# data61/gossamer

Measured on AMD Instinct MI355X. Metric: M k-mers/s (canonical, counted) at k=25, 150 bp reads, higher is better.
Workload: dtype u64

## Files before the change

### gossamer_amd/csrc/fused_path.hpp

```cpp
#pragma once

enum { kFusedDeclined = 0, kFusedDone = 1, kFusedNeedFull = 2, kFusedGoOn = -1, kFusedAgain = -2 };
constexpr uint32_t kFusedGrid = 256 * GOSS_E1_OCC;
#ifndef GOSS_FUSED_NKEYS2
#define GOSS_FUSED_NKEYS2 14
#endif
#ifndef GOSS_FUSED_GRID2
#define GOSS_FUSED_GRID2 512
#endif
constexpr uint32_t kFusedGrid2 = GOSS_FUSED_GRID2;
constexpr double kValidSlackA = 1.06, kValidSlackB = 1.17;
constexpr uint64_t kValidSizingMin = 640u << 20;

struct FusedForm {
    enum Table {
        kSmall,
        kBig,
        kWide,
        k96,
        kRem32
    };
    Table table = kSmall;
    uint32_t segbits = kSegBits;
    bool msd = false;
// ... 367 lines not shown
template <class F> void with_digit_hists(int nh, F&& f)
{
    if (nh == 0) f(std::integral_constant<int, 0>{});
    else if (nh == 1) f(std::integral_constant<int, 1>{});
    else f(std::integral_constant<int, 2>{});
}

struct FirstLevelLaunch {
    const uint8_t* d_bases; const uint8_t* aligned; const uint8_t* pk_src; const uint16_t* pk_bad;
    uint32_t mis; uint64_t nstarts, navail;
    void* ka; PartCounters* pc; const GapTable* dgt;
    uint32_t part_shift; uint64_t nsuper; uint32_t blk_log2, grid;
    int nh;
};

template <int MODE, int REPK>
void launch_extract1_part(goss_gpu_ctx* c, const FirstLevelLaunch& a, bool fastk, bool narrow, uint32_t nr_rbits, uint32_t nr_sqbit, uint32_t nr_dmask,
                          uint32_t nr_capg)
{
    with_digit_hists(a.nh, [&](auto nh_c) { with_bool(fastk, [&](auto fast_c) { with_bool(narrow, [&](auto narrow_c) {
        constexpr int NH = decltype(nh_c)::value;
        constexpr bool FAST = NH == 0 && decltype(fast_c)::value, NRW = NH == 0 && decltype(narrow_c)::value;
        if (c->rec_mode)
            hipLaunchKernelGGL(HIP_KERNEL_NAME(extract1_part_kernel<MODE, NH, REPK, true, FAST, NRW>), dim3(a.grid), dim3(kTB), 0, c->stream,
                               a.d_bases, 0u, a.nstarts, a.nstarts / rec_slots(c), c->len, (Key1*)a.ka, a.pc, a.dgt, a.part_shift, a.nsuper, a.blk_log2,
                               nr_rbits, nr_sqbit, nr_dmask, nr_capg);
        else if (c->pk.on)
            hipLaunchKernelGGL(HIP_KERNEL_NAME(extract1_part_kernel<MODE, NH, REPK, false, FAST, NRW, true>), dim3(a.grid), dim3(kTB), 0, c->stream,
                               a.pk_src, a.mis, a.nstarts, a.navail, c->len, (Key1*)a.ka, a.pc, a.dgt, a.part_shift, a.nsuper, a.blk_log2,
                               nr_rbits, nr_sqbit, nr_dmask, nr_capg, a.pk_bad);
        else
            hipLaunchKernelGGL(HIP_KERNEL_NAME(extract1_part_kernel<MODE, NH, REPK, false, FAST, NRW>), dim3(a.grid), dim3(kTB), 0, c->stream,
                               a.aligned, a.mis, a.nstarts, a.navail, c->len, (Key1*)a.ka, a.pc, a.dgt, a.part_shift, a.nsuper, a.blk_log2,
                               nr_rbits, nr_sqbit, nr_dmask, nr_capg, (const uint16_t*)nullptr);
    }); }); });
}

template <int MODE, int NBH>
void launch_extract2_part(goss_gpu_ctx* c, const FirstLevelLaunch& a)
{
    with_digit_hists(a.nh, [&](auto nh_c) {
        constexpr int NH = decltype(nh_c)::value;
        if constexpr (MODE == 0)
            if (c->rec_mode)
            {
                hipLaunchKernelGGL(HIP_KERNEL_NAME(extract2_part_kernel<0, NH, GOSS_FUSED_NKEYS2, NBH, true>), dim3(a.grid), dim3(kTB), 0, c->stream,
                                   a.d_bases, 0u, a.nstarts, a.nstarts / rec_slots(c), c->len, (Key2*)a.ka, a.pc, a.dgt, a.part_shift, a.nsuper, a.blk_log2);
                return;
            }
        if (c->pk.on)
            hipLaunchKernelGGL(HIP_KERNEL_NAME(extract2_part_kernel<MODE, NH, GOSS_FUSED_NKEYS2, NBH, false, true>), dim3(a.grid), dim3(kTB), 0, c->stream,
                               a.pk_src, a.mis, a.nstarts, a.navail, c->len, (Key2*)a.ka, a.pc, a.dgt, a.part_shift, a.nsuper, a.blk_log2, a.pk_bad);
        else
            hipLaunchKernelGGL(HIP_KERNEL_NAME(extract2_part_kernel<MODE, NH, GOSS_FUSED_NKEYS2, NBH>), dim3(a.grid), dim3(kTB), 0, c->stream,
                               a.aligned, a.mis, a.nstarts, a.navail, c->len, (Key2*)a.ka, a.pc, a.dgt, a.part_shift, a.nsuper, a.blk_log2,
                               (const uint16_t*)nullptr);
    });
}

template <class K>
void launch_first_level(const FusedChunk<K>& ch, const FusedForm& form, bool canon_l1, const BucketRegions& br, const GapTable* dgt, PartCounters* pc)
{
    goss_gpu_ctx* c = ch.c;
    const uint32_t shift = ch.keybits - form.segbits, npass = (form.segbits + 7) / 8;
    FirstLevelLaunch a{};
    const uintptr_t addr = (uintptr_t)ch.d_bases;
    a.d_bases = ch.d_bases;
    a.mis = (uint32_t)(addr & 15u);
    a.aligned = (const uint8_t*)(addr - a.mis);
    if (c->pk.on && !c->rec_mode) { pk_ptrs(c, a.aligned, &a.pk_src, &a.pk_bad); c->pk_fused_chunks++; }
    a.nstarts = ch.nstarts; a.navail = ch.navail;
    a.ka = ch.ka; a.pc = pc; a.dgt = dgt;
    a.part_shift = form.msd ? ch.keybits - 8 : shift;
    a.nsuper = (ch.nstarts + br.super - 1) / br.super;
    a.blk_log2 = br.blk_log2;
    a.grid = br.grid;
    a.nh = form.msd ? 0 : (npass > 2 ? 2 : 1);
    PhaseTimer t(c, GOSS_T_EXTRACT, ch.nstarts);
    if constexpr (FusedChunk<K>::kOne)
    {
        const bool fastk = a.nh == 0 && 2 * c->len >= 32 && a.part_shift >= 34 && !c->no_fast32;
        const bool narrow = form.msd && form.rem32() && form.narrow;
        const uint32_t nr_rbits = form.rbits32, nr_sqbit = form.squeeze ? c->len - 1 : 0u, nr_dmask = (1u << form.r32_bits) - 1u;
        const uint32_t nr_capg = std::min(656u, std::max(576u, c->narrow_capg));
        if (ch.graph_mode) launch_extract1_part<1, 0>(c, a, fastk, narrow, nr_rbits, nr_sqbit, nr_dmask, nr_capg);
        else if (canon_l1) launch_extract1_part<0, 2>(c, a, fastk, narrow, nr_rbits, nr_sqbit, nr_dmask, nr_capg);
        else if (c->len & 1u) launch_extract1_part<0, 1>(c, a, fastk, narrow, nr_rbits, nr_sqbit, nr_dmask, nr_capg);
        else launch_extract1_part<0, 0>(c, a, fastk, narrow, nr_rbits, nr_sqbit, nr_dmask, nr_capg);
    }
    else
    {
        if (ch.graph_mode) launch_extract2_part<1, 8>(c, a);
        else if (ch.rep_graph) launch_extract2_part<0, 0>(c, a);
        else
            switch (key2_nbh(c))
            {
                case 2: launch_extract2_part<0, 2>(c, a); break;
                case 4: launch_extract2_part<0, 4>(c, a); break;
                case 6: launch_extract2_part<0, 6>(c, a); break;
                default: launch_extract2_part<0, 8>(c, a); break;
            }
    }
    t.stop();
}

struct FirstLevelResult { uint64_t n = 0, tiles = 0, windows = 0; };

template <class K>
int read_first_level(const FusedChunk<K>& ch, const FusedForm& form, const BucketRegions& br, const PartCounters* pc, GapTable* gt, GapTable* dgt,
                     FirstLevelResult* out)
{
    goss_gpu_ctx* c = ch.c;
    std::vector<unsigned long long> hpc(sizeof(PartCounters) / 8);
    HIP_TRY(hipMemcpyAsync(hpc.data(), pc, sizeof(PartCounters), hipMemcpyDeviceToHost, c->stream));
    HIP_TRY(hipStreamSynchronize(c->stream));
    const PartCounters* hp = (const PartCounters*)hpc.data();
    if (hp->overflow) { c->fused_overflows++; return ch.decline("a bucket region overflowed"); }
    ch.lap("extraction + first level");
#if defined(GOSS_STAMPS)
    if (hp->hist[505])
        std::fprintf(stderr, "libgossgpu: stamps per tile (cycles): A %.0f  B %.0f  C %.0f  scatter %.0f  D %.0f   (%llu tiles)\n",
                     (double)hp->hist[500] / hp->hist[505], (double)hp->hist[501] / hp->hist[505], (double)hp->hist[502] / hp->hist[505],
                     (double)hp->hist[503] / hp->hist[505], (double)hp->hist[504] / hp->hist[505], (unsigned long long)hp->hist[505]);
    if (hp->hist[505] && hp->hist[506])
        std::fprintf(stderr, "libgossgpu: stamps, finer: C = scan %.0f + bookkeeping %.0f + barrier; scatter = LDS %.0f + encoder %.0f + barrier; D = stores %.0f + absorb %.0f + barrier %.0f\n",
                     (double)hp->hist[506] / hp->hist[505], (double)hp->hist[507] / hp->hist[505], (double)hp->hist[510] / hp->hist[505],
                     (double)hp->hist[511] / hp->hist[505], (double)hp->hist[508] / hp->hist[505], (double)hp->hist[509] / hp->hist[505],
                     (double)hp->hist[504] / hp->hist[505]);
#endif
    const uint64_t n = hp->keys_out;
    if (n == 0) return kFusedDeclined;
    if (n > ch.ka_slots || n > ch.kb_slots) return ch.decline("more keys than the buffers hold");
    const bool narrow = form.rem32() && form.narrow;
    uint64_t tiles = 0, sum = 0;
    const uint64_t tile_keys = narrow ? (uint64_t)(form.r32_bits == 9 ? Sub32N<9>::kTileSlots : Sub32N<10>::kTileSlots)
                             : form.rem32() ? (uint64_t)kSub32Tile : form.msd ? (uint64_t)SubCfg<K>::kTile : (uint64_t)SortCfg<K, false>::kTile;
    for (int d = 0; d < 256; ++d)
    {
        gt->cnt[d] = hp->cursors[d * kCursorStride];
        gt->tile_first[d] = tiles;
        tiles += (gt->cnt[d] + tile_keys - 1) / tile_keys;
        sum += gt->cnt[d];
    }
    gt->tile_first[256] = tiles;
    const uint64_t n_slots = narrow ? n / 3 * 2 : n;
    const uint64_t B = 1ULL << br.blk_log2;
    if (sum < n_slots || sum > n_slots + 8 + (uint64_t)br.grid * 256 * (2 * B + 8))
        throw StatusError{GOSS_ERR_HIP, "fused extraction: bucket counts do not add up"};
    HIP_TRY(hipMemcpyAsync(dgt, gt, sizeof(GapTable), hipMemcpyHostToDevice, c->stream));
    out->n = n; out->tiles = tiles; out->windows = hp->windows;
    return kFusedGoOn;
}

struct FusedLookback { LookbackCtl* ctl; LookbackCtl* hctl; };

inline int count_rem32(const FusedChunk<Key1>& ch, FusedForm form, const Sub32Regions& sub, const FirstLevelResult& fl, const GapTable* dgt,
                       FusedLookback lb, Run* r)
{
    goss_gpu_ctx* c = ch.c;
    Key1* ka = ch.ka; Key1* kb = ch.kb;
    const uint64_t n = fl.n, tiles = fl.tiles;
    const uint32_t r32_regions = form.r32_regions(), r32_bits = form.r32_bits, r32_split = form.r32_split, rbits32 = form.rbits32;
    const uint32_t sqbit32 = c->len - 1;
    const bool narrow = form.narrow, squeeze = form.squeeze;
    const bool image = r32_split == 0;
    if (squeeze && (rbits32 != kNarrowSqRbits || r32_bits != kNarrowSqDigitBits))
        throw StatusError{GOSS_ERR_HIP, "fused path: the squeeze form with other than 33-bit remainders under nine second-level bits"};
// ... 316 lines not shown
```

### gossamer_amd/csrc/goss_gpu.hip

```cpp
#include "../../include/goss_gpu.h"

#include <hip/hip_runtime.h>
#include <dlfcn.h>

#include <algorithm>
#include <chrono>
#include <cmath>
#include <cstdio>
#include <cstdlib>
#include <cstring>
#include <functional>
#include <map>
#include <mutex>
#include <string>
#include <system_error>
#include <thread>
#include <vector>

#include "goss_kernels.hpp"
#include "goss_reader.hpp"

using namespace goss;

namespace {
// ... 35 lines not shown
    void release(uint64_t m) { hi = m; }
    uint64_t avail() const { return hi > lo ? hi - lo : 0; }
};

struct OutFile {
    std::string suffix;
    uint64_t size = 0;
    const uint8_t* dev = nullptr;
    std::vector<uint8_t> host;
};

typedef std::map<std::pair<uint64_t, uint64_t>, uint64_t> BigMap;
struct Run { void* keys; uint32_t* counts; uint64_t m; int big = -1; bool rep = false; };

struct PhaseEvents { hipEvent_t a, b; int phase; uint64_t units; };

enum class Held : uint8_t { None, Segments, Entries, Components };
struct HeldResult { Held kind = Held::None; uint64_t lo = 0; };

constexpr double kCanonL1At = 0.05;
constexpr int kBigRoundsMax = 2;

}

struct goss_gpu_ctx {
    int device = 0;
    uint32_t k = 0, len = 0;
    int mode = 0;
    int words = 1;
    int path = 0;
    bool lookback = true;
    double est_scale = 1.0;
    uint32_t order_bits = 0;
    bool ordered_tiles = false;
    uint32_t lookback_failures = 0;
    uint64_t emit_estimate = 0;
    bool has_emit_estimate = false;
    struct Pending { hipEvent_t ev; void (*fn)(void*); void* user; };
    std::vector<Pending> pending;
    uint64_t flush_wait_us = 0, flush_count_us = 0, flushes = 0;
    struct PackedSrc { bool on = false; const uint32_t* codes = nullptr; const uint16_t* bad = nullptr; } pk;
    bool stage_pk[2] = {false, false};
    uint8_t* stage_buf[2] = {nullptr, nullptr};
    int stage_cur = 0;
    hipStream_t copy_stream = nullptr;
    std::thread bg;
    int bg_status = GOSS_OK;
    std::string bg_error;
    std::vector<hipEvent_t> pend_pool;
    uint8_t* stage = nullptr;
    uint64_t stage_cap = 0, stage_fill = 0;
    bool mute_timing = false;
    uint32_t segment_retries = 0;
    uint32_t extract_hist_shift = 0xFFFFFFFFu;
    bool extract_rep = false;
    uint32_t rep_chunks = 0;
    bool graph_rep = true;
    int canon_l1 = 1;
    bool more_follows = false;
    uint64_t more_starts = 0;
    uint64_t expect_bases = 0;
    int space_choice = -1;
    uint32_t canon_chunks = 0;
    bool fused = true;
    uint64_t fused_min = 32u << 20;
    uint32_t fused_overflows = 0;
    uint32_t valid_sized_chunks = 0;
    uint32_t valid_resizes = 0;
    uint64_t dump_lo = 0;
    bool dump_live = false;
    uint64_t budget_limit = 0;
    uint32_t arena_grows = 0;
    uint64_t arena_ms = 0;
    std::thread arena_thread;
    int arena_status = GOSS_OK;
    std::string arena_error;
    uint32_t seg_merges = 0;
    uint32_t hash_merges = 0;
    uint64_t hash_merge_min = 1u << 20;
    bool fused_msd = true;
    uint32_t fused_msd_chunks = 0;
    bool rem32 = true;
    int rem32_slots = 0;
    uint32_t narrow_capg = 656;
    bool narrow = true;
    uint32_t r32_small_max = 0;
    bool overflow_by_sort = true;
    uint64_t overflow_units = 0;
    uint32_t rem32_chunks = 0;
    uint32_t narrow_chunks = 0;
    uint64_t assemble_us = 0;
    uint64_t ds_blocks_ranges = 0, ds_blocks_own = 0;
    uint32_t pk_fused_chunks = 0;
    uint32_t pk_unpacked_chunks = 0;
    uint32_t rem32_bits_min = 0;
    uint32_t rem32_bits_last = 0;
    uint32_t rem32_split_min = 0;
    uint32_t rem32_split_last = 0;
    uint32_t fused_chunks = 0;
    bool debug = false;
    double fused_capscale = 1.0;
    uint32_t blk_log2_max = 0;
    bool no_fast32 = false;
    bool table96 = true;
    uint32_t table96_chunks = 0;
    bool wide_table = true;
    bool big_table = true;
    int big_rounds_min = 0;
    uint32_t big_table_chunks = 0;
    uint32_t wide_table_chunks = 0;
    bool rec_mode = false;
    uint32_t rec_chunks = 0;
    bool deferred = false;
    uint8_t* grp_send = nullptr;
    uint64_t grp_send_cap = 0;
    uint8_t* grp_inbox = nullptr;
    uint64_t grp_inbox_cap = 0;
    hipStream_t xstream = nullptr;
    double valid_frac = 1.0;
    bool size_by_valid = true;
    uint64_t budget = 0;
    hipStream_t stream = nullptr;
    bool own_stream = false;
    std::string last_error;
    Arena arena;
    std::vector<Run> runs;
    std::vector<BigMap> big_maps;
    BigMap res_big;
    bool pushed_counts = false;
    uint64_t windows = 0, keys_total = 0;
    bool finished = false, emitted = false;
    bool broken = false;
    double grp_count_ms = 0;
    void* res_keys = nullptr;
    uint32_t* res_counts = nullptr;
    uint64_t M = 0;
    void* tips_keys = nullptr;
    uint32_t* tips_counts = nullptr;
    HeldResult held;
    bool keep_held = false;
    void* seg_recs = nullptr;
    uint8_t* seg_text = nullptr;
    uint64_t seg_count = 0, seg_text_bytes = 0;
    uint32_t* cmp_marks = nullptr;
    uint64_t cmp_mark_words = 0, cmp_built_lo = 0, cmp_marked = 0;
    uint32_t* cmp_labels = nullptr;
    void* cmp_recs = nullptr;
    uint64_t cmp_count = 0;
    bool cmp_built = false;
    std::vector<OutFile> files;
    ExtractCounters* d_ctr = nullptr;
    uint32_t* d_flags = nullptr;
    void* d_route = nullptr;
    void* h_pinned = nullptr;
    std::vector<PhaseEvents> events;
    std::vector<hipEvent_t> event_pool;
    goss_gpu_timing timing{};
};

namespace {

struct PhaseTimer {
    goss_gpu_ctx* c;
    PhaseEvents pe;
    PhaseTimer(goss_gpu_ctx* ctx, int phase, uint64_t units = 0) : c(ctx)
    {
        muted = c->mute_timing;
// ... 5004 lines not shown
```

### gossamer_amd/csrc/kernels_extract.hpp

```cpp
#pragma once
#include <type_traits>

#include <hip/hip_runtime.h>
#include <stdint.h>

#include "goss_key.hpp"
#include "kernels_common.hpp"
#include "goss_words.hpp"

namespace goss {


struct ExtractCounters {
    unsigned long long keys_out;
    unsigned long long windows;
    unsigned long long hist[512];
};

template <bool PACKED = false>
__global__ __launch_bounds__(kTB) void nonbase_sample_kernel(const uint8_t* __restrict__ aligned, uint64_t nslices,
                                                             uint64_t stride, uint32_t slice,
                                                             unsigned long long* __restrict__ out)
{
    unsigned long long bad = 0, seen = 0;
// ... 343 lines not shown
        for (int g = 0; g < G; ++g)
        {
            const uint32_t vm = vmask[g];
            if (vm)
            {
                const uint32_t q0 = (g * kTB + tid) * P + mis;
                const uint32_t v0 = q0 >> 4, sh = q0 & 15u;
                const uint64_t w0 = (uint64_t)pk[v0] | ((uint64_t)pk[v0 + 1] << 32);
                const uint64_t w1 = (uint64_t)pk[v0 + 2] | ((uint64_t)pk[v0 + 3] << 32);
                const uint64_t w2 = (uint64_t)pk[v0 + 4] | ((uint64_t)pk[v0 + 5] << 32);
                uint32_t s = slot[g] * S;
                Key2 f{0, 0};
#pragma unroll
                for (int i = 0; i < P; ++i)
                {
                    const uint32_t t2 = 2 * (sh + i);
                    Key2 e;
                    e.lo = t2 ? ((w0 >> t2) | (w1 << (64 - t2))) : w0;
                    e.hi = (t2 ? ((w1 >> t2) | (w2 << (64 - t2))) : w1) & mask_hi;
                    if (i == 0)
                    {
                        const uint64_t rlo = rev64(e.hi), rhi = rev64(e.lo);
                        const uint32_t sft = 128 - bits;
                        if (sft == 64) { f.lo = rhi; f.hi = 0; }
                        else { f.lo = (rlo >> sft) | (rhi << (64 - sft)); f.hi = rhi >> sft; }
                    }
                    else
                    {
                        const uint32_t pos = 2 * (sh + i + len - 1);
                        const uint64_t nb = (pos < 64 ? (w0 >> pos) : pos < 128 ? (w1 >> (pos - 64)) : (w2 >> (pos - 128))) & 3u;
                        f.hi = ((f.hi << 2) | (f.lo >> 62)) & mask_hi;
                        f.lo = (f.lo << 2) | nb;
                    }
                    if ((vm >> i) & 1u)
                    {
                        const Key2 rk{~e.lo, (~e.hi) & mask_hi};
                        if (MODE == 0) { if constexpr (NBH == 0) stage[s++] = strand_rep2(f, rk, len, lmask); else stage[s++] = canonical_tail<NBH>(f, rk); }
                        else { stage[s++] = f; stage[s++] = rk; }
                    }
                }
            }
            __syncthreads();
            const uint32_t nk = sub_cnt[g] * S;
            for (uint32_t i = tid; i < nk; i += kTB) out[ob + i] = stage[i];
            ob += nk;
            __syncthreads();
        }
    }
}


constexpr int kCursorStride = 32;

struct GapTable {
    unsigned long long reg_start[256];
    unsigned long long reg_cap[256];
    unsigned long long cnt[256];
    unsigned long long tile_first[257];
};

struct PartCounters {
    unsigned long long keys_out, windows, overflow, pad;
    unsigned long long hist[512];
    unsigned long long cursors[256 * kCursorStride];
};

constexpr int kSubCursorStride = 4;
struct SubTable {
    unsigned long long start[65536];
    unsigned long long cap[65536];
};

constexpr uint64_t kPadKey = ~0ULL;

constexpr uint32_t kSkPadWord2 = 1u << 27;
__host__ __device__ inline uint32_t rec_windows(uint32_t w2) { return (w2 >> 27) == 1u ? 0u : (w2 >> 28) + 1u; }
#ifndef GOSS_E1_NK
#define GOSS_E1_NK 16
#endif
#ifndef GOSS_E1_OCC
#define GOSS_E1_OCC 3
#endif
#ifndef GOSS_E1_NCH
#define GOSS_E1_NCH 4
#endif
#ifndef GOSS_E1_PRIO_C
#define GOSS_E1_PRIO_C 1
#define GOSS_E1_PRIO_S 2
#define GOSS_E1_PRIO_E 1
#define GOSS_E1_PRIO_D 3
#endif
__device__ __forceinline__ uint32_t bit_select(uint32_t mask, uint32_t ones, uint32_t zeros)
{
    uint32_t d;
    asm("v_bfi_b32 %0, %1, %2, %3" : "=v"(d) : "v"(mask), "v"(ones), "v"(zeros));
    return d;
}
template <int MODE, int NH, int REPK, bool REC = false, bool FAST = false, bool NARROW = false, bool PACKED = false>
__global__ __launch_bounds__(kTB, GOSS_E1_OCC) void extract1_part_kernel(const uint8_t* __restrict__ bases_aligned, uint32_t mis,
                                                            uint64_t nstarts, uint64_t navail, uint32_t len,
                                                            Key1* __restrict__ out, PartCounters* __restrict__ pc,
                                                            const GapTable* __restrict__ gt, uint32_t shift, uint64_t nsuper,
                                                            uint32_t blk_log2, uint32_t nr_rbits = 0, uint32_t nr_sqbit = 0, uint32_t nr_dmask = 0, uint32_t nr_capg = 0,
                                                            const uint16_t* __restrict__ pbad = nullptr)
{
    static_assert(!(PACKED && REC), "records are not bases");
    static_assert(!NARROW || NH == 0, "the narrow form is the two-level form's");
    constexpr int S = MODE == 1 ? 2 : 1;
    constexpr int P = GOSS_E1_NK / S;
#if !defined(GOSS_E1_EXPERIMENT)
    static_assert(!REC || GOSS_E1_NK == 16, "a record of 16 windows holds at most one thread's first window");
#endif
    constexpr int T = kTB * P;
    constexpr int NVEC = T / 16 + 4;
    constexpr int NK = P * S;
    constexpr int kCarry = NARROW ? 11 : 7;
    constexpr uint32_t kGran = NARROW ? 12 : 8;
    constexpr uint32_t kSlots = NARROW ? 656 * 12 : T * S + 256 * kCarry;
    static_assert(kSlots % kGran == 0 && kSlots >= T * S + 256 * kCarry, "whole granules, and room for a tile without carried keys");
    constexpr uint32_t kGarb = kSlots;
    constexpr int kPairs = GOSS_E1_NK >= 16 ? 5 : 3;
    constexpr uint32_t kStep = 2 * kPairs * kTB;
    constexpr uint32_t kNG = NARROW ? 772 : kSlots / kGran + 4;
    constexpr uint32_t kSkip = 0xFFFFFFFFu;
    constexpr uint32_t kSortedBytes = NARROW ? (kSlots + 128) * 6 : (kSlots + 128) * 8;
    constexpr uint32_t kDigBase = (kSlots + 128) * 4;
    static_assert(kDigBase % 16 == 0, "the digit array starts on a 16-byte boundary");
    __shared__ __attribute__((aligned(64))) unsigned char lds_all[kSortedBytes + (288 + 288 + kNG + 8 + (NH ? 256 * NH : 0)) * 4];
    Key1* const sorted = reinterpret_cast<Key1*>(lds_all);
    uint32_t* const dh = reinterpret_cast<uint32_t*>(lds_all + kSortedBytes);
    uint32_t* const tab = dh + 288;
    uint32_t* const gaddr = tab + 288;
    uint32_t* const sh_scan = gaddr + kNG;
    uint32_t& sh_ovf = sh_scan[6];
    uint32_t* const lh = sh_scan + 8;
    uint32_t* pk = reinterpret_cast<uint32_t*>(sorted);
    uint32_t* iv = pk + NVEC;

    const uint32_t tid = threadIdx.x;
    if (NH > 0) lh[tid] = 0;
    if (NH > 1) lh[tid + 256] = 0;
    dh[tid] = 0;
    if (tid < 32) { dh[256 + tid] = 0; tab[256 + tid] = kGarb << (NARROW ? 2 : 3); }
    if (tid == 0) { sh_ovf = 0; gaddr[kSlots / kGran] = kSkip; }
    const uint64_t my_start = gt->reg_start[tid], my_cap = gt->reg_cap[tid];
    const uint32_t B = 1u << blk_log2;
    const uint32_t bits = 2 * len;
    const uint64_t kmask = (1ULL << bits) - 1;
    const uint64_t lmask = (1ULL << len) - 1;
    unsigned long long nvalid = 0;
    uint64_t wpos = 0;
    uint32_t ccnt = 0;
    Key1 kc[NARROW ? 1 : kCarry];
#pragma unroll
    for (int j = 0; j < (NARROW ? 1 : kCarry); ++j) kc[j].lo = 0;
    uint4 clo0 = make_uint4(0, 0, 0, 0), clo1 = clo0, clo2 = clo0;
    uint64_t cdig0 = 0, cdig1 = 0, cdig2 = 0;
    [[maybe_unused]] auto store_short_granule = [&](Key1* at) {
        const uint32_t lw[12] = {clo0.x, clo0.y, clo0.z, clo0.w, clo1.x, clo1.y, clo1.z, clo1.w, clo2.x, clo2.y, clo2.z, clo2.w};
        const uint64_t dw[3] = {cdig0, cdig1, cdig2};
        uint4* const g = reinterpret_cast<uint4*>(at);
#pragma unroll
        for (int c = 0; c < 4; ++c)
        {
            const uint32_t nv = ccnt > (uint32_t)c + 8 ? 3u : ccnt > (uint32_t)c + 4 ? 2u : ccnt > (uint32_t)c ? 1u : 0u;
            const uint32_t da = (uint32_t)(dw[c / 4] >> (16 * (c % 4))) & 0x3FFu;
            const uint32_t db = (uint32_t)(dw[(c + 4) / 4] >> (16 * ((c + 4) % 4))) & 0x3FFu;
            const uint32_t dc = (uint32_t)(dw[(c + 8) / 4] >> (16 * ((c + 8) % 4))) & 0x3FFu;
            g[c] = make_uint4(lw[c], lw[c + 4], lw[c + 8], da | (db << 10) | (dc << 20) | (nv << 30));
        }
    };

    auto fetch = [&](uint64_t byte0, uint4& q) -> bool {
        if constexpr (PACKED)
        {
            q = make_uint4(0u, 0xFFFFu, 0u, 0u);
            if (byte0 < navail + mis)
            {
                const uint64_t g = byte0 >> 4;
                q.x = reinterpret_cast<const uint32_t*>(bases_aligned)[g];
                q.y = pbad[g];
                const uint64_t left = navail + mis - byte0;
                q.z = left < 16 ? (0xFFFFu << (uint32_t)left) & 0xFFFFu : 0u;
            }
            return true;
        }
        if (byte0 + 16 <= navail + mis) { q = *reinterpret_cast<const uint4*>(bases_aligned + byte0); return true; }
        q = make_uint4(0x0A0A0A0Au, 0x0A0A0A0Au, 0x0A0A0A0Au, 0x0A0A0A0Au);
        if (byte0 < navail + mis)
        {
            uint32_t w[4] = {q.x, q.y, q.z, q.w};
            for (int j = 0; j < 16; ++j)
            {
                uint64_t b = byte0 + j;
                uint32_t c = b < navail + mis ? bases_aligned[b] : 0x0Au;
                w[j >> 2] = (w[j >> 2] & ~(0xFFu << (8 * (j & 3)))) | (c << (8 * (j & 3)));
            }
            q = make_uint4(w[0], w[1], w[2], w[3]);
        }
        return true;
    };
    auto encode = [](const uint4& q, uint32_t& codes, uint32_t& bads) {
        if constexpr (PACKED) { codes = q.x; bads = q.y | q.z; return; }
        const uint32_t w[4] = {q.x, q.y, q.z, q.w};
        codes = 0; bads = 0;
#pragma unroll
        for (int i = 0; i < 4; ++i)
        {
            uint32_t bad;
            const uint32_t x = base_codes(w[i], bad);
            codes |= pack_codes(x) << (8 * i);
            bads |= pack_flags(bad) << (4 * i);
        }
    };
    constexpr uint32_t NV0 = T / 16;
    static_assert(NVEC == NV0 + 4 && NV0 <= kTB, "one vector per thread and four more");
    uint32_t c0 = 0, b0 = 0, c1 = 0, b1 = 0;
    const uint32_t* recw = reinterpret_cast<const uint32_t*>(bases_aligned);
    const uint64_t nrec = navail;
    uint64_t rc_next = 0, rc_end = 0;
    uint32_t ra0 = 0, ra1 = 0, ra2 = kSkPadWord2, rb0 = 0, rb1 = 0, rb2 = kSkPadWord2;
    uint32_t* rbuf = pk;
    uint32_t* rmark = pk + 512 * 8;
    auto stage_rec = [&](uint32_t at, uint32_t x0, uint32_t x1, uint32_t x2, uint32_t before) {
        const uint32_t x2m = x2 & 0x0FFFFFFFu, nw = (x2 >> 28) + 1u;
        if constexpr (!(MODE == 0 && REPK == 1))
        {
// ... 209 lines not shown
#pragma unroll
                for (int i = 0; i < P; ++i)
                {
                    const uint32_t t2 = 30u - r_s2;
                    const uint32_t rlo = __builtin_amdgcn_alignbit(rc1, rc0, r_s2) & kmlo, rhi = __builtin_amdgcn_alignbit(rc2, rc1, r_s2) & kmhi;
                    const uint32_t flo = __builtin_amdgcn_alignbit(rv1, rv0, t2) & kmlo, fhi = __builtin_amdgcn_alignbit(rv2, rv1, t2) & kmhi;
                    if (MODE == 0 && REPK == 1)
                    {
                        const uint32_t sel = (uint32_t)__builtin_amdgcn_sbfe((int32_t)flo, len - 1u, 1u);
                        kreg[i].lo = ((uint64_t)bit_select(sel, rhi, fhi) << 32) | bit_select(sel, rlo, flo);
                    }
                    else emit(i, ((uint64_t)fhi << 32) | flo, ((uint64_t)rhi << 32) | rlo);
                    if (i + 1 < P)
                    {
                        r_s2 += 2u;
                        if (r_s2 >= r_nw2 && r_at < 511) next_rec();
                    }
                }
            }
            else if constexpr (FAST)
            {
                constexpr bool kLoose = MODE == 0 && REPK == 1 && NARROW && NH == 0;
                [[maybe_unused]] const uint32_t kmhi = (uint32_t)(kmask >> 32);
                const uint32_t cw0 = ~(uint32_t)blo, cw1 = ~(uint32_t)(blo >> 32), cw2 = ~(uint32_t)bhi;
                const uint32_t pn = bits - 2;
                const uint32_t nx = (uint32_t)((blo >> pn) | (bhi << (64 - pn)));
                const uint32_t mid = (uint32_t)(blo >> (len - 1));
                const uint64_t f0 = rev64(blo & kmask) >> (64 - bits);
                uint32_t flo = (uint32_t)f0, fhi = (uint32_t)(f0 >> 32);
#pragma unroll
                for (int i = 0; i < P; ++i)
                {
                    if (i)
                    {
                        const uint32_t nb = (nx >> (2 * i)) & 3u;
                        fhi = __builtin_amdgcn_alignbit(fhi, flo, 30);
                        if constexpr (!kLoose) fhi &= kmhi;
                        flo = (flo << 2) | nb;
                    }
                    const uint32_t rlo = i ? __builtin_amdgcn_alignbit(cw1, cw0, 2 * i) : cw0;
                    uint32_t rhi = i ? __builtin_amdgcn_alignbit(cw2, cw1, 2 * i) : cw1;
                    if constexpr (!kLoose) rhi &= kmhi;
                    if (MODE == 0 && REPK == 1)
                    {
                        const uint32_t sel = (uint32_t)__builtin_amdgcn_sbfe((int32_t)mid, 2 * i, 1);
                        kreg[i].lo = ((uint64_t)bit_select(sel, rhi, fhi) << 32) | bit_select(sel, rlo, flo);
                    }
                    else emit(i, ((uint64_t)fhi << 32) | flo, ((uint64_t)rhi << 32) | rlo);
#pragma unroll
                    for (int u = 0; u < S; ++u) rank_key(i * S + u);
                }
            }
            else
            {
                uint64_t f = rev64(blo & kmask) >> (64 - bits);
                uint64_t r = (~blo) & kmask;
                const uint32_t top = bits - 2;
#pragma unroll
                for (int i = 0; i < P; ++i)
                {
                    if (i)
                    {
                        const uint32_t pos = 2 * (i + len - 1);
                        const uint32_t nb = (uint32_t)(pos < 64 ? (blo >> pos) : (bhi >> (pos - 64))) & 3u;
                        f = ((f << 2) | nb) & kmask;
                        r = (r >> 2) | ((uint64_t)(nb ^ 3u) << top);
                    }
                    emit(i, f, r);
                }
            }
            if constexpr (REC || !FAST)
            {
#pragma unroll
                for (int j = 0; j < NK; ++j) rank_key(j);
            }
        }
        __syncthreads();
        GOSS_STAMP(1);
#if !defined(GOSS_E1_NOPRIO)
        __builtin_amdgcn_s_setprio(GOSS_E1_PRIO_C);
#endif

        uint32_t total_slots = 0, part_at = 0, absorb = 0;
        if constexpr (NARROW)
        {
            const uint32_t cnt = dh[tid];
            uint32_t tot = ccnt + cnt;
            uint32_t fg = (tot * 0xAAABu) >> 19;
            uint32_t rest = tot - 12u * fg;
            uint32_t g_at = block_excl_scan_open_u32(fg + (rest ? 1u : 0u), sh_scan, &total_slots);
            GOSS_STAMP(6);
            dh[tid] = 0;
            if (tid < 32) dh[256 + tid] = 0;
            uint32_t thr, tbx, tby;
            auto take_room = [&](uint32_t fl) {
                const uint32_t room = (B - ((uint32_t)wpos & (B - 1))) & (B - 1);
                thr = fl;
                tbx = (uint32_t)(wpos >> 3);
                tby = 0;
                if (fl > room)
                {
                    thr = room;
                    const uint32_t need = fl - room;
                    unsigned long long at, want;
                    if (has_resv && need <= B) { at = resv; want = B; has_resv = false; }
                    else
                    {
                        want = ((uint64_t)(need + B - 1) >> blk_log2) << blk_log2;
                        at = atomicAdd(&pc->cursors[tid * kCursorStride], want);
                    }
                    if (at + want > my_cap) { atomicOr(&pc->overflow, 1ULL); sh_ovf = 1; }
                    tby = (uint32_t)((my_start + at) >> 3);
                    wpos = my_start + at + need;
                }
                else wpos += fl;
            };
            if (total_slots > nr_capg)
            {
                if (ccnt)
                {
                    take_room(8u);
                    if (sh_ovf == 0) store_short_granule(out + ((uint64_t)(thr ? tbx : tby) << 3));
                    ccnt = 0;
                }
                __syncthreads();
                tot = cnt;
                fg = (tot * 0xAAABu) >> 19;
                rest = tot - 12u * fg;
                g_at = block_excl_scan_open_u32(fg + (rest ? 1u : 0u), sh_scan, &total_slots);
            }
            const uint32_t fl = fg << 3;
            part_at = 12u * (g_at + fg);
            take_room(fl);
            tab[tid] = (12u * g_at + ccnt) << 2;
            {
                const uint32_t t8 = thr >> 3;
                const uint32_t yb = tby - t8;
#pragma unroll
                for (uint32_t g = 0; g < 3; ++g)
                    if (g < fg) gaddr[g_at + g] = (g < t8 ? tbx : yb) + g;
#pragma clang loop unroll(disable) vectorize(disable) interleave(disable)
                for (uint32_t g = 3; g < fg; ++g) gaddr[g_at + g] = (g < t8 ? tbx : yb) + g;
                if (rest) gaddr[g_at + fg] = kSkip;
            }
            if (ccnt)
            {
                unsigned char* const lp = lds_all + 48u * g_at;
                unsigned char* const dp = lds_all + kDigBase + 24u * g_at;
                reinterpret_cast<uint4*>(lp)[0] = clo0; reinterpret_cast<uint4*>(lp)[1] = clo1; reinterpret_cast<uint4*>(lp)[2] = clo2;
                reinterpret_cast<uint64_t*>(dp)[0] = cdig0; reinterpret_cast<uint64_t*>(dp)[1] = cdig1; reinterpret_cast<uint64_t*>(dp)[2] = cdig2;
            }
            ccnt = rest;
        }
        else
        {
            const uint32_t cnt = dh[tid];
            const uint32_t a8 = cnt & ~7u, b = cnt & 7u;
            const uint32_t s_at = block_excl_scan_open_u32((cnt + 7u) & ~7u, sh_scan, &total_slots);
            GOSS_STAMP(6);
            dh[tid] = 0;
            if (tid < 32) dh[256 + tid] = 0;
            const bool top = b + ccnt >= 8u;
            const uint32_t take = top ? 8u - b : 0u;
            const uint32_t fl = a8 + (top ? 8u : 0u);
            absorb = top ? 0u : b;
            part_at = s_at + a8;
            const uint32_t room = (B - ((uint32_t)wpos & (B - 1))) & (B - 1);
            uint32_t thr = fl;
            const uint32_t tbx = (uint32_t)(wpos >> 3);
            uint32_t tby = 0;
            if (fl > room)
            {
                thr = room;
                const uint32_t need = fl - room;
                unsigned long long at, want;
                if (has_resv && need <= B) { at = resv; want = B; has_resv = false; }
                else
                {
                    want = ((uint64_t)(need + B - 1) >> blk_log2) << blk_log2;
                    at = atomicAdd(&pc->cursors[tid * kCursorStride], want);
                }
                if (at + want > my_cap) { atomicOr(&pc->overflow, 1ULL); sh_ovf = 1; }
                tby = (uint32_t)((my_start + at) >> 3);
                wpos = my_start + at + need;
            }
            else wpos += fl;
            tab[tid] = s_at << 3;
            {
                const uint32_t g0 = s_at >> 3, ng = fl >> 3, t8 = thr >> 3;
                const uint32_t yb = tby - t8;
#pragma unroll
                for (uint32_t g = 0; g < 4; ++g)
                    if (g < ng) gaddr[g0 + g] = (g < t8 ? tbx : yb) + g;
#pragma clang loop unroll(disable) vectorize(disable) interleave(disable)
                for (uint32_t g = 4; g < ng; ++g) gaddr[g0 + g] = (g < t8 ? tbx : yb) + g;
                if (absorb) gaddr[g0 + ng] = kSkip;
            }
            {
                const uint32_t from = ccnt - take;
#pragma unroll
                for (int j = 0; j < kCarry; ++j)
                    sorted[((uint32_t)j >= from && (uint32_t)j < ccnt ? part_at + b - from : kGarb + (tid & 63u)) + j] = kc[j];
                ccnt = from;
            }
        }
        GOSS_STAMP(7);
        __syncthreads();
        GOSS_STAMP(2);
#if !defined(GOSS_E1_NOPRIO)
        __builtin_amdgcn_s_setprio(GOSS_E1_PRIO_S);
#endif
        {
            uint32_t tb[NK];
#pragma unroll
            for (int i = 0; i < NK; ++i) tb[i] = *reinterpret_cast<const uint32_t*>(reinterpret_cast<const char*>(tab) + bin4[i]);
            if constexpr (NARROW)
            {
                auto put = [&](auto sq_tag, auto hi_tag) {
                    constexpr bool kSq = decltype(sq_tag)::value, kHi = decltype(hi_tag)::value;
                    const uint32_t lomask = kSq ? (1u << nr_sqbit) - 1u : (nr_rbits >= 32 ? 0xFFFFFFFFu : (1u << nr_rbits) - 1u);
                    const uint32_t dbits = (uint32_t)__popc(nr_dmask);
#pragma unroll
                    for (int i = 0; i < NK; ++i)
                    {
                        const uint32_t klo = (uint32_t)kreg[i].lo, khi = (uint32_t)(kreg[i].lo >> 32);
                        uint32_t rem, dg;
                        if constexpr (kSq && kHi)
                        {
                            rem = klo;
                            dg = narrow_sq_field(khi);
                        }
                        else
                        {
                            rem = klo & lomask;
                            if (kSq) rem |= __builtin_amdgcn_alignbit(khi, klo, nr_sqbit + 1u) << nr_sqbit;
                            dg = kHi ? __builtin_amdgcn_ubfe(khi, nr_rbits - 32u, dbits)
                                     : (__builtin_amdgcn_alignbit(khi, klo, nr_rbits) & nr_dmask);
                        }
                        const uint32_t la = tb[i] + (rk[i] << 2);
                        *reinterpret_cast<uint32_t*>(lds_all + la) = rem;
                        *reinterpret_cast<uint16_t*>(lds_all + kDigBase + (la >> 1)) = (uint16_t)dg;
                    }
                };
                if (nr_sqbit) { if (nr_rbits >= 32) put(std::true_type{}, std::true_type{}); else put(std::true_type{}, std::false_type{}); }
                else { if (nr_rbits >= 32) put(std::false_type{}, std::true_type{}); else put(std::false_type{}, std::false_type{}); }
            }
            else
#pragma unroll
            for (int i = 0; i < NK; ++i)
            {
                *reinterpret_cast<Key1*>(reinterpret_cast<char*>(sorted) + (tb[i] + (rk[i] << 3))) = kreg[i];
                if (NH > 0)
                {
                    const bool ok = (vm >> (i / S)) & 1u;
                    const Key1 k = kreg[i];
                    atomicAdd(&lh[(uint32_t)(k.lo >> (shift + 8)) & 0xFFu], ok ? 1u : 0u);
                    if (NH > 1) atomicAdd(&lh[256u + ((uint32_t)(key_shr64(k, shift + 16)) & 0xFFu)], ok ? 1u : 0u);
                }
            }
        }
        GOSS_STAMP(10);
#if !defined(GOSS_E1_NOPRIO)
        __builtin_amdgcn_s_setprio(GOSS_E1_PRIO_E);
#endif
        if (more && !REC)
        {
            encode(q0, c0, b0);
            if (tid < 4) encode(q1, c1, b1);
        }
        GOSS_STAMP(11);
        if constexpr (REC) asm volatile("" ::"v"(ra0), "v"(ra1), "v"(ra2), "v"(rb0), "v"(rb1), "v"(rb2));
        __syncthreads();
        GOSS_STAMP(3);
#if !defined(GOSS_E1_NOPRIO)
        __builtin_amdgcn_s_setprio(GOSS_E1_PRIO_D);
#endif

        if constexpr (NARROW)
        {
            {
                const unsigned char* const lp = lds_all + 4u * part_at;
                const unsigned char* const dp = lds_all + kDigBase + 2u * part_at;
                clo0 = reinterpret_cast<const uint4*>(lp)[0]; clo1 = reinterpret_cast<const uint4*>(lp)[1]; clo2 = reinterpret_cast<const uint4*>(lp)[2];
                cdig0 = reinterpret_cast<const uint64_t*>(dp)[0]; cdig1 = reinterpret_cast<const uint64_t*>(dp)[1]; cdig2 = reinterpret_cast<const uint64_t*>(dp)[2];
            }
            if (sh_ovf == 0)
            {
                constexpr int kCh = GOSS_E1_NCH;
                static_assert(kSlots / 12u * 4u <= 2624u + 64u && kCh == 4, "the reads past the layout stay inside the allocation (kNG)");
                const uint32_t nchunk = total_slots << 2;
                const uint32_t c = tid & 3u;
                Key1* const lane_out = out + 2u * c;
                const unsigned char* lp = lds_all + (12u * tid - 8u * c);
                const unsigned char* dp = lds_all + kDigBase + (6u * tid - 4u * c);
                const unsigned char* gp = reinterpret_cast<const unsigned char*>(gaddr) + (tid & ~3u);
                for (uint32_t base = 0; base < nchunk; base += kCh * kTB, lp += 12u * kCh * kTB, dp += 6u * kCh * kTB, gp += kCh * kTB)
                {
                    uint32_t r0[kCh], r1[kCh], r2[kCh], d0[kCh], d1[kCh], d2[kCh], ga[kCh];
#pragma unroll
                    for (int u = 0; u < kCh; ++u)
                    {
                        r0[u] = *reinterpret_cast<const uint32_t*>(lp + 3072 * u);
                        r1[u] = *reinterpret_cast<const uint32_t*>(lp + 3072 * u + 16);
                        r2[u] = *reinterpret_cast<const uint32_t*>(lp + 3072 * u + 32);
                        d0[u] = *reinterpret_cast<const uint16_t*>(dp + 1536 * u);
                        d1[u] = *reinterpret_cast<const uint16_t*>(dp + 1536 * u + 8);
                        d2[u] = *reinterpret_cast<const uint16_t*>(dp + 1536 * u + 16);
                        ga[u] = *reinterpret_cast<const uint32_t*>(gp + 256 * u);
                    }
#pragma unroll
                    for (int u = 0; u < kCh; ++u) asm volatile("" : "+v"(r0[u]), "+v"(r1[u]), "+v"(r2[u]), "+v"(d0[u]), "+v"(d1[u]), "+v"(d2[u]), "+v"(ga[u]));
                    const uint32_t left = nchunk - base;
#pragma unroll
                    for (int u = 0; u < kCh; ++u)
                    {
                        const uint4 ch = make_uint4(r0[u], r1[u], r2[u], d0[u] | (d1[u] << 10) | (d2[u] << 20) | (3u << 30));
                        if (ga[u] != kSkip && tid + u * kTB < left) *reinterpret_cast<uint4*>(lane_out + ((uint64_t)ga[u] << 3)) = ch;
                    }
                }
            }
            GOSS_STAMP(8);
            GOSS_STAMP(9);
        }
        else
        {
        Key1 ab[kCarry];
#pragma unroll
        for (int j = 0; j < kCarry; ++j)
        {
            const bool in = (uint32_t)j >= ccnt && (uint32_t)j < ccnt + absorb;
            ab[j] = sorted[in ? part_at + j - ccnt : kGarb];
        }
        if (sh_ovf == 0)
        {
            Key1* const lane_out = out + ((2 * tid) & 7u);
            for (uint32_t base = 0; base < total_slots; base += kStep)
            {
                uint4 kk[kPairs];
                uint32_t ga[kPairs];
#pragma unroll
                for (int u = 0; u < kPairs; ++u)
                {
                    const uint32_t i = min(base + 2 * (tid + u * kTB), kSlots);
                    kk[u] = *reinterpret_cast<const uint4*>(&sorted[i]);
                    ga[u] = gaddr[i >> 3];
                }
#pragma unroll
                for (int u = 0; u < kPairs; ++u) asm volatile("" : "+v"(kk[u].x), "+v"(kk[u].y), "+v"(kk[u].z), "+v"(kk[u].w), "+v"(ga[u]));
#pragma unroll
                for (int u = 0; u < kPairs; ++u)
                {
#if defined(GOSS_E1_EXP) && GOSS_E1_EXP == 1
                    asm volatile("" ::"v"(kk[u].x), "v"(kk[u].y), "v"(kk[u].z), "v"(kk[u].w), "v"(ga[u]));
#elif defined(GOSS_E1_EXP) && GOSS_E1_EXP == 2
                    if (ga[u] != kSkip && (ga[u] % 3u) != 0u && base + 2 * (tid + u * kTB) < total_slots) *reinterpret_cast<uint4*>(lane_out + ((uint64_t)ga[u] << 3)) = kk[u];
#else
                    if (ga[u] != kSkip && base + 2 * (tid + u * kTB) < total_slots) *reinterpret_cast<uint4*>(lane_out + ((uint64_t)ga[u] << 3)) = kk[u];
#endif
                }
            }
        }
        GOSS_STAMP(8);
        {
#pragma unroll
            for (int j = 0; j < kCarry; ++j)
            {
                const bool in = (uint32_t)j >= ccnt && (uint32_t)j < ccnt + absorb;
                kc[j] = in ? ab[j] : kc[j];
            }
            ccnt += absorb;
        }
        GOSS_STAMP(9);
        }
        __syncthreads();
        GOSS_STAMP(4);
    }
#if defined(GOSS_STAMPS)
    if (tid == 0)
        for (int i = 0; i < 12; ++i) atomicAdd(&pc->hist[500 + i], st_acc[i]);
#endif
#undef GOSS_STAMP

    if (sh_ovf == 0)
    {
        bool spare_blk = has_resv;
        if (ccnt)
        {
            const uint32_t room = (B - ((uint32_t)wpos & (B - 1))) & (B - 1);
            if (room == 0)
            {
                unsigned long long at;
                if (has_resv) { at = resv; spare_blk = false; }
                else at = atomicAdd(&pc->cursors[tid * kCursorStride], (unsigned long long)B);
                if (at + B > my_cap) { atomicOr(&pc->overflow, 1ULL); ccnt = 0; wpos = 0; }
                else wpos = my_start + at;
            }
            if constexpr (NARROW)
            {
                if (ccnt)
                {
// ... 589 lines not shown
```

Before: 182,100.

## Compact narrow-form write list to full granules and enlarge LDS layout

```diff
diff --git a/gossamer_amd/csrc/fused_path.hpp b/gossamer_amd/csrc/fused_path.hpp
--- a/gossamer_amd/csrc/fused_path.hpp
+++ b/gossamer_amd/csrc/fused_path.hpp
@@ -473,7 +473,7 @@
         const bool fastk = a.nh == 0 && 2 * c->len >= 32 && a.part_shift >= 34 && !c->no_fast32;
         const bool narrow = form.msd && form.rem32() && form.narrow;
         const uint32_t nr_rbits = form.rbits32, nr_sqbit = form.squeeze ? c->len - 1 : 0u, nr_dmask = (1u << form.r32_bits) - 1u;
-        const uint32_t nr_capg = std::min(656u, std::max(576u, c->narrow_capg));
+        const uint32_t nr_capg = std::max(576u, c->narrow_capg);
         if (ch.graph_mode) launch_extract1_part<1, 0>(c, a, fastk, narrow, nr_rbits, nr_sqbit, nr_dmask, nr_capg);
         else if (canon_l1) launch_extract1_part<0, 2>(c, a, fastk, narrow, nr_rbits, nr_sqbit, nr_dmask, nr_capg);
         else if (c->len & 1u) launch_extract1_part<0, 1>(c, a, fastk, narrow, nr_rbits, nr_sqbit, nr_dmask, nr_capg);
diff --git a/gossamer_amd/csrc/goss_gpu.hip b/gossamer_amd/csrc/goss_gpu.hip
--- a/gossamer_amd/csrc/goss_gpu.hip
+++ b/gossamer_amd/csrc/goss_gpu.hip
@@ -141,7 +141,7 @@
     uint32_t fused_msd_chunks = 0;
     bool rem32 = true;
     int rem32_slots = 0;
-    uint32_t narrow_capg = 656;
+    uint32_t narrow_capg = 0xFFFFFFFFu;
     bool narrow = true;
     uint32_t r32_small_max = 0;
     bool overflow_by_sort = true;
diff --git a/gossamer_amd/csrc/kernels_extract.hpp b/gossamer_amd/csrc/kernels_extract.hpp
--- a/gossamer_amd/csrc/kernels_extract.hpp
+++ b/gossamer_amd/csrc/kernels_extract.hpp
@@ -449,7 +449,7 @@
 #define GOSS_E1_OCC 3
 #endif
 #ifndef GOSS_E1_NCH
-#define GOSS_E1_NCH 4
+#define GOSS_E1_NCH 5
 #endif
 #ifndef GOSS_E1_PRIO_C
 #define GOSS_E1_PRIO_C 1
@@ -483,21 +483,35 @@
     constexpr int NK = P * S;
     constexpr int kCarry = NARROW ? 11 : 7;
     constexpr uint32_t kGran = NARROW ? 12 : 8;
-    constexpr uint32_t kSlots = NARROW ? 656 * 12 : T * S + 256 * kCarry;
+    constexpr uint32_t kListMax = (T * S + 256 * 11) / 12;
+    constexpr uint32_t kListN = (kListMax + 64 * GOSS_E1_NCH - 1) / (64 * GOSS_E1_NCH) * (64 * GOSS_E1_NCH);
+    constexpr uint32_t kLdsBudget = 53760;
+    constexpr uint32_t kTabBytes = (288 + 288 + 8) * 4;
+    constexpr uint32_t kListBytes = NARROW ? kListN * 2 + kListMax * 4 : 0;
+    static_assert(kLdsBudget > kListBytes + kTabBytes + 128 * 6, "the list and the tables leave room for a layout");
+    constexpr uint32_t kLayG = ((kLdsBudget - kListBytes - kTabBytes) / 6 - 128) / 12;
+    constexpr uint32_t kSlots = NARROW ? kLayG * 12 : T * S + 256 * kCarry;
     static_assert(kSlots % kGran == 0 && kSlots >= T * S + 256 * kCarry, "whole granules, and room for a tile without carried keys");
+    static_assert(kSlots / kGran + 256 < 65536 && (T * S + 256 * kCarry) / kGran + 256 < 65536, "both sums of the packed scan stay below 2^16");
+    static_assert(!NARROW || (kSlots / 12 - 1) * 24 < 65536, "a granule's digit offset is a 16-bit list entry");
+    static_assert((kListN - kListMax) * 4 <= 2 * 288 * 4, "the reads past the list's addresses stay inside dh and tab");
     constexpr uint32_t kGarb = kSlots;
     constexpr int kPairs = GOSS_E1_NK >= 16 ? 5 : 3;
     constexpr uint32_t kStep = 2 * kPairs * kTB;
-    constexpr uint32_t kNG = NARROW ? 772 : kSlots / kGran + 4;
-    constexpr uint32_t kSkip = 0xFFFFFFFFu;
+    constexpr uint32_t kNG = NARROW ? 0 : kSlots / kGran + 4;
+    [[maybe_unused]] constexpr uint32_t kSkip = 0xFFFFFFFFu;
     constexpr uint32_t kSortedBytes = NARROW ? (kSlots + 128) * 6 : (kSlots + 128) * 8;
     constexpr uint32_t kDigBase = (kSlots + 128) * 4;
     static_assert(kDigBase % 16 == 0, "the digit array starts on a 16-byte boundary");
-    __shared__ __attribute__((aligned(64))) unsigned char lds_all[kSortedBytes + (288 + 288 + kNG + 8 + (NH ? 256 * NH : 0)) * 4];
+    static_assert(kSortedBytes % 4 == 0 && kListBytes % 4 == 0, "the list and the tables behind it are arrays of words");
+    __shared__ __attribute__((aligned(64))) unsigned char lds_all[kSortedBytes + kListBytes + kTabBytes + (kNG + (NH ? 256 * NH : 0)) * 4];
+    static_assert(!NARROW || sizeof(lds_all) <= kLdsBudget, "three workgroups per CU");
     Key1* const sorted = reinterpret_cast<Key1*>(lds_all);
-    uint32_t* const dh = reinterpret_cast<uint32_t*>(lds_all + kSortedBytes);
+    [[maybe_unused]] uint16_t* const lgl = reinterpret_cast<uint16_t*>(lds_all + kSortedBytes);
+    [[maybe_unused]] uint32_t* const gal = reinterpret_cast<uint32_t*>(lds_all + kSortedBytes + (NARROW ? kListN * 2 : 0));
+    uint32_t* const dh = reinterpret_cast<uint32_t*>(lds_all + kSortedBytes + kListBytes);
     uint32_t* const tab = dh + 288;
-    uint32_t* const gaddr = tab + 288;
+    [[maybe_unused]] uint32_t* const gaddr = tab + 288;
     uint32_t* const sh_scan = gaddr + kNG;
     uint32_t& sh_ovf = sh_scan[6];
     uint32_t* const lh = sh_scan + 8;
@@ -509,7 +523,12 @@
     if (NH > 1) lh[tid + 256] = 0;
     dh[tid] = 0;
     if (tid < 32) { dh[256 + tid] = 0; tab[256 + tid] = kGarb << (NARROW ? 2 : 3); }
-    if (tid == 0) { sh_ovf = 0; gaddr[kSlots / kGran] = kSkip; }
+    if (tid == 0) sh_ovf = 0;
+    if constexpr (NARROW)
+    {
+        for (uint32_t j = tid; j < kListN / 2; j += kTB) reinterpret_cast<uint32_t*>(lgl)[j] = 0;
+    }
+    else if (tid == 0) gaddr[kSlots / kGran] = kSkip;
     const uint64_t my_start = gt->reg_start[tid], my_cap = gt->reg_cap[tid];
     const uint32_t B = 1u << blk_log2;
     const uint32_t bits = 2 * len;
@@ -885,13 +904,16 @@
 #endif
 
         uint32_t total_slots = 0, part_at = 0, absorb = 0;
+        [[maybe_unused]] uint32_t whole = 0;
         if constexpr (NARROW)
         {
             const uint32_t cnt = dh[tid];
             uint32_t tot = ccnt + cnt;
             uint32_t fg = (tot * 0xAAABu) >> 19;
             uint32_t rest = tot - 12u * fg;
-            uint32_t g_at = block_excl_scan_open_u32(fg + (rest ? 1u : 0u), sh_scan, &total_slots);
+            uint32_t both = 0;
+            uint32_t at2 = block_excl_scan_open_u32(((fg + (rest ? 1u : 0u)) | (fg << 16)), sh_scan, &both);
+            total_slots = both & 0xFFFFu;
             GOSS_STAMP(6);
             dh[tid] = 0;
             if (tid < 32) dh[256 + tid] = 0;
@@ -918,7 +940,7 @@
                 }
                 else wpos += fl;
             };
-            if (total_slots > nr_capg)
+            if (total_slots > min(nr_capg, kSlots / 12u))
             {
                 if (ccnt)
                 {
@@ -930,8 +952,11 @@
                 tot = cnt;
                 fg = (tot * 0xAAABu) >> 19;
                 rest = tot - 12u * fg;
-                g_at = block_excl_scan_open_u32(fg + (rest ? 1u : 0u), sh_scan, &total_slots);
-            }
+                at2 = block_excl_scan_open_u32(((fg + (rest ? 1u : 0u)) | (fg << 16)), sh_scan, &both);
+                total_slots = both & 0xFFFFu;
+            }
+            whole = both >> 16;
+            const uint32_t g_at = at2 & 0xFFFFu, w_at = at2 >> 16;
             const uint32_t fl = fg << 3;
             part_at = 12u * (g_at + fg);
             take_room(fl);
@@ -941,10 +966,9 @@
                 const uint32_t yb = tby - t8;
 #pragma unroll
                 for (uint32_t g = 0; g < 3; ++g)
-                    if (g < fg) gaddr[g_at + g] = (g < t8 ? tbx : yb) + g;
+                    if (g < fg) { gal[w_at + g] = (g < t8 ? tbx : yb) + g; lgl[w_at + g] = (uint16_t)(24u * (g_at + g)); }
 #pragma clang loop unroll(disable) vectorize(disable) interleave(disable)
-                for (uint32_t g = 3; g < fg; ++g) gaddr[g_at + g] = (g < t8 ? tbx : yb) + g;
-                if (rest) gaddr[g_at + fg] = kSkip;
+                for (uint32_t g = 3; g < fg; ++g) { gal[w_at + g] = (g < t8 ? tbx : yb) + g; lgl[w_at + g] = (uint16_t)(24u * (g_at + g)); }
             }
             if (ccnt)
             {
@@ -1090,26 +1114,37 @@
             if (sh_ovf == 0)
             {
                 constexpr int kCh = GOSS_E1_NCH;
-                static_assert(kSlots / 12u * 4u <= 2624u + 64u && kCh == 4, "the reads past the layout stay inside the allocation (kNG)");
-                const uint32_t nchunk = total_slots << 2;
-                const uint32_t c = tid & 3u;
-                Key1* const lane_out = out + 2u * c;
-                const unsigned char* lp = lds_all + (12u * tid - 8u * c);
-                const unsigned char* dp = lds_all + kDigBase + (6u * tid - 4u * c);
-                const unsigned char* gp = reinterpret_cast<const unsigned char*>(gaddr) + (tid & ~3u);
-                for (uint32_t base = 0; base < nchunk; base += kCh * kTB, lp += 12u * kCh * kTB, dp += 6u * kCh * kTB, gp += kCh * kTB)
-                {
-                    uint32_t r0[kCh], r1[kCh], r2[kCh], d0[kCh], d1[kCh], d2[kCh], ga[kCh];
+                static_assert(kListN % (64 * kCh) == 0 && kListN >= kListMax, "whole rounds of entries: no read past lgl");
+                const uint32_t nchunk = whole << 2;
+                uint32_t t = tid;
+                asm volatile("" : "+v"(t));
+                const uint32_t c2 = (t & 3u) << 1;
+                Key1* const lane_out = out + c2;
+                const unsigned char* ep = reinterpret_cast<const unsigned char*>(lgl) + ((t >> 2) << 1);
+                const unsigned char* gp = reinterpret_cast<const unsigned char*>(gal) + (t & ~3u);
+                for (uint32_t base = 0; base < nchunk; base += kCh * kTB, gp += kCh * kTB, ep += kCh * kTB / 2)
+                {
+                    uint32_t r0[kCh], r1[kCh], r2[kCh], d0[kCh], d1[kCh], d2[kCh], ga[kCh], lo[kCh];
 #pragma unroll
                     for (int u = 0; u < kCh; ++u)
                     {
-                        r0[u] = *reinterpret_cast<const uint32_t*>(lp + 3072 * u);
-                        r1[u] = *reinterpret_cast<const uint32_t*>(lp + 3072 * u + 16);
-                        r2[u] = *reinterpret_cast<const uint32_t*>(lp + 3072 * u + 32);
-                        d0[u] = *reinterpret_cast<const uint16_t*>(dp + 1536 * u);
-                        d1[u] = *reinterpret_cast<const uint16_t*>(dp + 1536 * u + 8);
-                        d2[u] = *reinterpret_cast<const uint16_t*>(dp + 1536 * u + 16);
+                        lo[u] = *reinterpret_cast<const uint16_t*>(ep + 128 * u);
                         ga[u] = *reinterpret_cast<const uint32_t*>(gp + 256 * u);
+                    }
+#pragma unroll
+                    for (int u = 0; u < kCh; ++u) asm volatile("" : "+v"(lo[u]));
+#pragma unroll
+                    for (int u = 0; u < kCh; ++u)
+                    {
+                        const uint32_t x = lo[u] + c2;
+                        const unsigned char* const dp = lds_all + kDigBase + x;
+                        const unsigned char* const lp = lds_all + 2u * x;
+                        r0[u] = *reinterpret_cast<const uint32_t*>(lp);
+                        r1[u] = *reinterpret_cast<const uint32_t*>(lp + 16);
+                        r2[u] = *reinterpret_cast<const uint32_t*>(lp + 32);
+                        d0[u] = *reinterpret_cast<const uint16_t*>(dp);
+                        d1[u] = *reinterpret_cast<const uint16_t*>(dp + 8);
+                        d2[u] = *reinterpret_cast<const uint16_t*>(dp + 16);
                     }
 #pragma unroll
                     for (int u = 0; u < kCh; ++u) asm volatile("" : "+v"(r0[u]), "+v"(r1[u]), "+v"(r2[u]), "+v"(d0[u]), "+v"(d1[u]), "+v"(d2[u]), "+v"(ga[u]));
@@ -1118,7 +1153,7 @@
                     for (int u = 0; u < kCh; ++u)
                     {
                         const uint4 ch = make_uint4(r0[u], r1[u], r2[u], d0[u] | (d1[u] << 10) | (d2[u] << 20) | (3u << 30));
-                        if (ga[u] != kSkip && tid + u * kTB < left) *reinterpret_cast<uint4*>(lane_out + ((uint64_t)ga[u] << 3)) = ch;
+                        if (tid + u * kTB < left) *reinterpret_cast<uint4*>(lane_out + ((uint64_t)ga[u] << 3)) = ch;
                     }
                 }
             }
```

Result: faster. 187,600, median of 6 (+3.0%).
